# kanster/moped

Hardware: AMD Instinct MI355X
Metric: detections/sec (frames/s) 640x480 ~3k SIFT vs N models (higher is better)
Workload: dtype f32

## Files before the change

moped_amd/csrc/match_screen.hip:

```cpp
#include <type_traits>
#include <hip/hip_fp16.h>

#include <algorithm>
#include <cstdlib>

#include "common.h"
#include "screen.h"

MH_TRACE_TU()

namespace mh {

namespace {

typedef _Float16 half8 __attribute__((ext_vector_type(8)));
typedef float v16f __attribute__((ext_vector_type(16)));
#define MH_AS1 __attribute__((address_space(1)))
#define MH_AS3 __attribute__((address_space(3)))

constexpr int SC_QPAD = 3 * 1024;
constexpr int SC_TILE = 128;
constexpr int SC_TILE_BYTES = SC_TILE * DIM * 2;
constexpr bool SC_SHAPE16_LARGE = true;
constexpr int SC_NW_LARGE = 8;
// ... 141 lines not shown
      const float qq = qnorm[row];
      bad = (!(qq >= 0.f) || qq == __builtin_inff() || !(m < 60000.f)) ? 1 : 0;
      if (qq == -1.f) bad = 2;
      else if (!bad && m == 0.f && qq == 0.f) bad = 3;
    }
    qbad[row] = (uint8_t)bad;
  }
}

constexpr int SC_SLOTS_MAX = 256;
constexpr int SC_SA_SLOTS = 32;
constexpr int SC_SLOT_PITCH = SC_SLOTS_MAX + SC_SA_SLOTS;

#ifdef SC_PROF
__device__ unsigned long long g_sc_prof[8];
__device__ unsigned long long g_sc_trace[2][1024];
static int g_sc_ablate = 0;
#define SC_ABL(bit) ((A.ablate >> (bit)) & 1)
#define SC_EV(e) do { if (tracing && n_ev < 1024) { g_sc_trace[wave >> 2][n_ev++] = ((unsigned long long)(e) << 56) | (__builtin_amdgcn_s_memtime() - t_start); } } while (0)
#else
#define SC_ABL(bit) 0
#define SC_EV(e) do { } while (0)
#endif

struct ScreenArgs {
  const _Float16* qh;
  const _Float16* dbh;
  const float* dneg;
  const float* qnorm;
  const uint8_t* qbad;
  const int32_t* q_count;
  float2* part;
  float* part5;
  const float* tau;
  uint2* recs;
  int32_t* ovf_cnt;
  uint2* ovf;
  int Q, q_pad, ovf_cap, sub_cap;
  int n_sel, tile_first, tile_stride;
  int tiles_base, tiles_rem, n_splits;
  int n_splits_a;
  unsigned pack_keep;
  int skip_first, skip_stride;
  float dmax;
  int ablate;
};
// ... 23 lines not shown
  }
  tau[q] = t;
}

constexpr int SC_TOPK = 4;
constexpr int SC_PART5 = SC_TOPK + 1;
constexpr int SC_SA_SPLITS_MAX = 28;
constexpr int SC_PACK_BITS_MAX = 10;
constexpr float SC_PACK_FLOOR = -1e38f;
constexpr unsigned SC_REC_LAYOUT16 = 0x80000000u;
constexpr unsigned SC_REC_SAMPLE = 0x40000000u;

struct SampleGeom {
  int sa_slots;
  int pack_bits;
  int tile_first, tile_stride, tiles_base, tiles_rem, n_sel;
};

constexpr int HO_PARTS_MAX = 16;
template <int HS>
__global__ __launch_bounds__(64 * HO_PARTS_MAX) void screen_handover_kernel(
    const float* __restrict__ part5, int n_lane_slots, int q_pad, int Q, const int32_t* __restrict__ q_count,
    const float* __restrict__ qnorm, const uint8_t* __restrict__ qbad, float dmax, SampleGeom g, float* __restrict__ tau,
    uint2* __restrict__ recs, unsigned int* __restrict__ inc) {
  MH_TRACE_SCOPE(mh::TK_TAU);
  __shared__ float s_b[HO_PARTS_MAX][64], s_s[HO_PARTS_MAX][64];
  __shared__ int s_cnt[HO_PARTS_MAX][64];
  __shared__ unsigned s_sm[64], s_qm[64];
  const int ql = threadIdx.x, part = threadIdx.y, n_parts = blockDim.y;
  const int q = blockIdx.x * 64 + ql;
  const int Qe = q_count ? min(Q, *q_count) : Q;
  const bool live = q < q_pad && q < Qe && !qbad[q];
  const int ls0 = part * HS;
  float v[HS][SC_PART5];
#pragma unroll
  for (int j = 0; j < HS; ++j)
#pragma unroll
    for (int k = 0; k < SC_PART5; ++k)
      v[j][k] = live && ls0 + j < n_lane_slots ? part5[((size_t)(ls0 + j) * SC_PART5 + k) * q_pad + q] : -__builtin_inff();
  const float qq = live ? qnorm[q] : 0.f;
  if (part == 0) {
    s_sm[ql] = 0u;
    s_qm[ql] = 0u;
  }
  float B = -__builtin_inff(), S = -__builtin_inff();
#pragma unroll
  for (int j = 0; j < HS; ++j) {
// ... 35 lines not shown
#pragma unroll
  for (int j = 0; j < HS; ++j) {
    const int ls = ls0 + j;
    const bool swept = ((sm >> (ls >> 2)) & 1u) && ((qm >> (ls & 3)) & 1u);
    n_j[j] = 0;
    bool run = hand && !swept;
#pragma unroll
    for (int k = 0; k < SC_TOPK; ++k) {
      run = run && v[j][k] > thr;
      n_j[j] += run ? 1 : 0;
    }
    cnt += n_j[j];
  }
  s_cnt[part][ql] = cnt;
  __syncthreads();
  int before = 0, total = 0;
  for (int p = 0; p < n_parts; ++p) {
    const int c = s_cnt[p][ql];
    before += p < part ? c : 0;
    total += c;
  }
  const bool full = total > g.sa_slots;
  if (cnt && !full) {
    uint2* mine = recs + (size_t)q * SC_SLOT_PITCH + SC_SLOTS_MAX + before;
    const unsigned id_mask = (1u << g.pack_bits) - 1u;
    int n = 0;
#pragma unroll
    for (int j = 0; j < HS; ++j) {
      const int split = (ls0 + j) >> 2, quarter = (ls0 + j) & 3;
#pragma unroll
      for (int k = 0; k < SC_TOPK; ++k)
        if (k < n_j[j]) {
          const unsigned id = __float_as_uint(v[j][k]) & id_mask;
          const int sel = split * g.tiles_base + min(split, g.tiles_rem) + (int)(id >> 2);
          const unsigned row0 = (unsigned)((g.tile_first + sel * g.tile_stride) * SC_TILE + (int)(id & 3u) * 32 + 4 * quarter);
          mine[n++] = make_uint2(row0 | SC_REC_LAYOUT16 | SC_REC_SAMPLE, 0xFFu | ((unsigned)screen_record_value(v[j][k], t) << 16));
        }
    }
  }
  if (part == 0 && q < q_pad) {
    if (full) {
      sm = (1u << (n_lane_slots >> 2)) - 1u;
      qm = 0xFu;
    }
    tau[q] = t;
    if (inc) inc[q] = sm ? sm | (qm << 28) : 0u;
  }
}

__device__ __forceinline__ void dma16x4(unsigned voff, const void* b0, const void* b1, const void* b2, const void* b3,
                                        unsigned l0, unsigned l1, unsigned l2, unsigned l3) {
  unsigned keep;
  asm volatile(
      "s_mov_b32 %0, m0\n\t"
      "s_mov_b32 m0, %6\n\ts_nop 0\n\tglobal_load_lds_dwordx4 %1, %2\n\t"
      "s_mov_b32 m0, %7\n\ts_nop 0\n\tglobal_load_lds_dwordx4 %1, %3\n\t"
      "s_mov_b32 m0, %8\n\ts_nop 0\n\tglobal_load_lds_dwordx4 %1, %4\n\t"
      "s_mov_b32 m0, %9\n\ts_nop 0\n\tglobal_load_lds_dwordx4 %1, %5\n\t"
      "s_mov_b32 m0, %0"
      : "=&s"(keep)
      : "v"(voff), "s"(b0), "s"(b1), "s"(b2), "s"(b3), "s"(l0), "s"(l1), "s"(l2), "s"(l3)
      : "memory");
}
__device__ __forceinline__ void dma4(unsigned voff, const void* base, unsigned lds_dst) {
  unsigned keep;
  asm volatile("s_mov_b32 %0, m0\n\ts_mov_b32 m0, %3\n\ts_nop 0\n\tglobal_load_lds_dword %1, %2\n\ts_mov_b32 m0, %0"
               : "=&s"(keep) : "v"(voff), "s"(base), "s"(lds_dst) : "memory");
}
// ... 336 lines not shown
      const int jj = sel_begin - A.skip_first;
      tile_cur = sel_begin + 1 + jj / d;
      gap_cur = d - jj % d;
    }
  }
  auto stage = [&](int tile, int buf) {
    const unsigned char* tb = reinterpret_cast<const unsigned char*>(A.dbh) + (size_t)tile * SC_TILE_BYTES;
    const unsigned l = lds_base + buf * SC_TILE_BYTES + wave * 1024;
    dma16x4(voff, tb, tb + 8192, tb + 16384, tb + 24576, l, l + 8192, l + 16384, l + 24576);
    if (wave < 3)
      dma4(voff_dd, A.dneg + (size_t)tile * SC_DD, lds_base + SC_NBUF * SC_TILE_BYTES + buf * (SC_DD * 4) + wave * 256);
  };
  if (sel_begin < sel_end) stage(tile_cur, 0);
  half8 bq[NQB][2][4];
#pragma unroll
  for (int nb = 0; nb < NQB; ++nb)
#pragma unroll
    for (int tj = 0; tj < 2; ++tj) {
      const _Float16* row = A.qh + (size_t)(q0 + nb * 32 + 16 * tj + l16) * DIM + 8 * quarter;
#pragma unroll
      for (int s = 0; s < 4; ++s) bq[nb][tj][s] = *reinterpret_cast<const half8*>(row + 32 * s);
    }
  float pk[NQB][2][SC_PART5];
  unsigned n_rec[(NQB + 1) / 2] = {};
  float* const tau_lds = reinterpret_cast<float*>(lds + SC_LDS16_TAU) + wave * 128;
#pragma unroll
  for (int nb = 0; nb < NQB; ++nb)
#pragma unroll
    for (int tj = 0; tj < 2; ++tj)
#pragma unroll
      for (int k = 0; k < SC_PART5; ++k) pk[nb][tj][k] = -__builtin_inff();
  if (MODE == 1)
    for (int i = lane; i < QW; i += 64) tau_lds[i] = A.tau[q0 + i];
  __builtin_amdgcn_s_waitcnt(0x0F70);
  __syncthreads();

  uint4* const recbuf = reinterpret_cast<uint4*>(lds + SC_LDS_TILES + wave * (SC_RECBUF16 * SC_REC16_BYTES));
  int n_parked = 0;
  auto record_bits8 = [](const v4f& d0, const v4f& d1, float top, float thr) {
    unsigned bits = 0;
#pragma unroll
    for (int r = 3; r >= 0; --r) bits = __builtin_amdgcn_alignbit(bits, __float_as_uint(thr - d1[r]), 31);
#pragma unroll
    for (int r = 3; r >= 0; --r) bits = __builtin_amdgcn_alignbit(bits, __float_as_uint(thr - d0[r]), 31);
    return (bits & 0xFFu) | ((unsigned)screen_record_value(top, thr) << 16);
  };
  auto emit = [&](const v4f& d0, const v4f& d1, unsigned& nrec_word, int shift, int q, int row0, float top, float thr, int pos) {
    const int nrec = (int)((nrec_word >> shift) & 0xFFu);
    if (nrec < A.sub_cap) {
      const unsigned dst = (unsigned)q * SC_SLOT_PITCH + (4 * split + quarter) * A.sub_cap + nrec;
      nrec_word += 1u << shift;
      if (pos < SC_RECBUF16) {
        uint4* e = recbuf + 3 * pos;
        e[0] = make_uint4(dst, (unsigned)row0, __float_as_uint(thr), __float_as_uint(top));
        e[1] = make_uint4(__float_as_uint(d0[0]), __float_as_uint(d0[1]), __float_as_uint(d0[2]), __float_as_uint(d0[3]));
        e[2] = make_uint4(__float_as_uint(d1[0]), __float_as_uint(d1[1]), __float_as_uint(d1[2]), __float_as_uint(d1[3]));
      } else {
        A.recs[dst] = make_uint2((unsigned)row0 | SC_REC_LAYOUT16, record_bits8(d0, d1, top, thr));
      }
    } else {
      const int opos = atomicAdd(&A.ovf_cnt[q], 1);
      if (opos < A.ovf_cap) A.ovf[(size_t)q * A.ovf_cap + opos] = make_uint2((unsigned)row0 | SC_REC_LAYOUT16, record_bits8(d0, d1, top, thr));
      if (pos < SC_RECBUF16) recbuf[3 * pos] = make_uint4(0xFFFFFFFFu, 0u, 0u, 0u);
    }
  };
  auto emit_block = [&](bool hit0, bool hit1, const v4f (&p)[2][2], int nb, int row0, float m0, float m1, float thr0, float thr1) {
    const unsigned long long h0 = __ballot(hit0), h1 = __ballot(hit1);
    if ((h0 | h1) == 0ull) return;
    if (hit0)
      emit(p[0][0], p[1][0], n_rec[nb >> 1], 16 * (nb & 1), q0 + nb * 32 + l16, row0, m0, thr0,
           n_parked + (int)__builtin_amdgcn_mbcnt_hi((unsigned)(h0 >> 32), __builtin_amdgcn_mbcnt_lo((unsigned)h0, 0u)));
    n_parked += __popcll(h0);
    if (hit1)
      emit(p[0][1], p[1][1], n_rec[nb >> 1], 16 * (nb & 1) + 8, q0 + nb * 32 + 16 + l16, row0, m1, thr1,
           n_parked + (int)__builtin_amdgcn_mbcnt_hi((unsigned)(h1 >> 32), __builtin_amdgcn_mbcnt_lo((unsigned)h1, 0u)));
    n_parked += __popcll(h1);
  };
  auto flush_parked = [&]() {
    __builtin_amdgcn_fence(__ATOMIC_RELEASE, "wavefront");
    __builtin_amdgcn_wave_barrier();
    __builtin_amdgcn_fence(__ATOMIC_ACQUIRE, "wavefront");
    const int n = min(n_parked, SC_RECBUF16);
    for (int j = lane; j < n; j += 64) {
      const uint4 e = recbuf[3 * j];
      if (e.x == 0xFFFFFFFFu) continue;
      const uint4 x0 = recbuf[3 * j + 1], x1 = recbuf[3 * j + 2];
      const v4f d0 = {__uint_as_float(x0.x), __uint_as_float(x0.y), __uint_as_float(x0.z), __uint_as_float(x0.w)};
      const v4f d1 = {__uint_as_float(x1.x), __uint_as_float(x1.y), __uint_as_float(x1.z), __uint_as_float(x1.w)};
      A.recs[e.x] = make_uint2(e.y | SC_REC_LAYOUT16, record_bits8(d0, d1, __uint_as_float(e.w), __uint_as_float(e.z)));
    }
    __builtin_amdgcn_wave_barrier();
    n_parked = 0;
  };

  auto load_rb = [&](const unsigned char* T, int rb, half8 (&a)[2][4]) {
#pragma unroll
    for (int ti = 0; ti < 2; ++ti) {
      const unsigned char* rowp = T + (rb * 32 + 16 * ti + l16) * 256;
#pragma unroll
      for (int s = 0; s < 4; ++s) a[ti][s] = *reinterpret_cast<const half8*>(rowp + (((4 * s + quarter) ^ l16) << 4));
    }
  };
  auto max3 = [](float a, float b, float c) {
    float r;
    asm("v_max3_f32 %0, %1, %2, %3" : "=v"(r) : "v"(a), "v"(b), "v"(c));
    return r;
  };
  auto max8 = [&](const v4f& x, const v4f& y) {
    return max3(max3(max3(x[0], x[1], x[2]), x[3], y[0]), max3(y[1], y[2], y[3]), -__builtin_inff());
  };
  auto max8x2_after_mfma = [](const v4f (&acc)[2][2], float floor, float& m0, float& m1) {
    float t0, t1;
    asm("s_nop 7\n\ts_nop 7\n\t"
// ... 246 lines not shown
  int ovf_cap;
  float dmax;
  const float* tau;
  float spread;
  int32_t* idx1;
  float* d1;
  float* d2;
  unsigned int* stats;
  int32_t zero_idx;
  float zero_d1, zero_d2;
  SampleGeom g;
  const unsigned int* inc;
  unsigned int* inc_count;
  const _Float16* dbh;
  const float* dneg;
};
typedef const __attribute__((address_space(4))) RsArgs* RsArgsPtr;
__device__ __forceinline__ RsArgsPtr rs_args() {
  RsArgsPtr p = (RsArgsPtr)__builtin_amdgcn_kernarg_segment_ptr();
  asm volatile("" : "+s"(p));
  return p;
}

__device__ __forceinline__ void rs_load_slots(const uint2* recs, int n_slots, int sa_slots, int q, int lane, uint2 (&rv)[RS_ITERS]) {
  const uint2* theirs = recs + (size_t)q * SC_SLOT_PITCH;
  const int n_own = n_slots + sa_slots;
#pragma unroll
  for (int it = 0; it < RS_ITERS; ++it) {
    const int j = it * 64 + lane;
    rv[it] = j < n_own ? theirs[j < n_slots ? j : SC_SLOTS_MAX + (j - n_slots)] : make_uint2(0u, 0u);
  }
}
#define RS_CONST(T, p) ((const __attribute__((address_space(4))) T*)(p))
__device__ __forceinline__ RsScalars rs_load_scalars(const uint8_t* qbad, const float* qnorm, const float* tau, const int32_t* ovf_cnt,
                                                     const unsigned int* inc, const float* qn, int q, int lane) {
  RsScalars v;
  v.qv = reinterpret_cast<const float2*>(qn + (size_t)q * DIM)[lane];
  v.n_ovf = RS_CONST(int32_t, ovf_cnt)[q];
  const unsigned w = RS_CONST(unsigned int, inc ? inc : reinterpret_cast<const unsigned int*>(tau))[q];
  v.bad = (RS_CONST(unsigned int, qbad)[q >> 2] >> (8 * (q & 3))) & 0xFFu;
  v.nq = RS_CONST(float, qnorm)[q];
  v.tau_q = RS_CONST(float, tau)[q];
  v.incw = inc ? w : 0u;
  return v;
}

__device__ __forceinline__ void rescore_query(
    int q, int lane, float* q_sw, int* cand_sw, int* samp_sw, int* ncand_sw, int* nsamp_sw, uint2 (&recv)[RS_ITERS], const RsScalars sc, int Qe,
    const float* __restrict__ db, const float* __restrict__ dnorm, int N,
    RowMap rmap, uint2* __restrict__ recs, int n_slots, int32_t* __restrict__ ovf_cnt, uint2* __restrict__ ovf,
    int ovf_cap, float dmax, float spread, int32_t* __restrict__ idx1, float* __restrict__ d1, float* __restrict__ d2,
    unsigned int* __restrict__ stats, int32_t zero_idx, float zero_d1, float zero_d2, SampleGeom g,
    unsigned int* __restrict__ inc_count, const _Float16* __restrict__ dbh, const float* __restrict__ dneg) {
  uint2* mine = recs + (size_t)q * SC_SLOT_PITCH;
  const int n_own = n_slots + g.sa_slots;
  auto slot_at = [&](int j) -> uint2& { return mine[j < n_slots ? j : SC_SLOTS_MAX + (j - n_slots)]; };
  const int bad = sc.bad;
  const float nq = sc.nq;
  const float tau_q = sc.tau_q;
  const int n_ovf = sc.n_ovf;
  const unsigned incw = sc.incw;
  const float2 qv = sc.qv;
  asm volatile("" ::"v"(bad), "v"(nq), "v"(tau_q), "v"(n_ovf), "v"(incw), "v"(qv.x), "v"(qv.y), "s"(Qe));
  if (q >= Qe) {
    if (lane == 0) {
      idx1[q] = -1;
      d1[q] = __builtin_inff();
      d2[q] = __builtin_inff();
    }
    return;
  }
  if (bad == 2) {
    if (lane == 0) {
      idx1[q] = -1;
      d1[q] = __builtin_inff();
      d2[q] = __builtin_inff();
    }
    return;
  }
  if (bad == 3) {
    if (lane == 0) {
      idx1[q] = zero_idx >= 0 ? row_to_global(rmap, zero_idx) : -1;
      d1[q] = zero_d1;
      d2[q] = zero_d2;
      if (stats) stats[3 * q + 2] += 1u;
    }
    return;
  }
  wave_lds_sync();
  if (lane == 0) {
    *ncand_sw = 0;
    *nsamp_sw = 0;
  }
  q_sw[2 * lane] = qv.x;
  q_sw[2 * lane + 1] = qv.y;
  bool brute = n_ovf > ovf_cap || bad == 1;
  int n_cand = 0;
  if (!brute) {
    float l1 = -__builtin_inff(), l2 = -__builtin_inff();
    const float pert = screen_pack_pert(nq, dmax, g.pack_bits);
    auto bounds = [tau_q, spread, N, dmax, pert](uint2 rec, float& lo, float& hi) {
      if (rec.x & SC_REC_SAMPLE) screen_sample_bounds((unsigned short)(rec.y >> 16), tau_q, pert, dmax, lo, hi);
      else screen_record_bounds((unsigned short)(rec.y >> 16), rec.x & 0x3FFFFFFFu, tau_q, spread, N, dmax, lo, hi);
    };
#pragma unroll
    for (int it = 0; it < RS_ITERS; ++it) {
      const int j = it * 64 + lane;
      uint2 rec = recv[it];
      if (j < n_own) {
        if (rec.y) slot_at(j) = make_uint2(0u, 0u);
      } else if (j < n_own + n_ovf) {
        rec = ovf[(size_t)q * ovf_cap + (j - n_own)];
      }
      recv[it] = rec;
      if (rec.y & 0xFFFFu) {
        float lo, hi;
        bounds(rec, lo, hi);
        l2 = fmaxf(l2, fminf(l1, lo));
        l1 = fmaxf(l1, lo);
      }
    }
#pragma unroll
    for (int d = 1; d < 64; d <<= 1) {
      const float o1 = __shfl_xor(l1, d), o2 = __shfl_xor(l2, d);
      l2 = fmaxf(fmaxf(l2, o2), fminf(l1, o1));
      l1 = fmaxf(l1, o1);
    }
    const float keep_from = l2 - screen_margin(nq, dmax);
#pragma unroll
    for (int it = 0; it < RS_ITERS; ++it) {
      const uint2 rec = recv[it];
      unsigned bits = rec.y & 0xFFFFu;
      if (bits) {
        float lo, hi;
        bounds(rec, lo, hi);
        if (hi < keep_from) bits = 0;
      }
      const int hi_stride = (rec.x & 0x80000000u) ? 16 : 8;
      const int row0 = (int)(rec.x & 0x3FFFFFFFu);
      if (bits && (rec.x & SC_REC_SAMPLE)) {
        const int w = atomicAdd(nsamp_sw, 1);
        if (w < SC_SA_SLOTS) samp_sw[w] = row0;
        bits = 0;
      }
      while (bits) {
        const int r = __builtin_ctz(bits);
        bits &= bits - 1;
        const int w = atomicAdd(ncand_sw, 1);
        if (w < RS_MAXC) cand_sw[w] = row0 + (r & 3) + hi_stride * (r >> 2);
      }
    }
    wave_lds_sync();
    const int n_samp = min(*nsamp_sw, SC_SA_SLOTS), n_pad_rows = (N + SC_TILE - 1) / SC_TILE * SC_TILE;
    for (int p = 0; p < n_samp; p += 2) {
      const bool pair = p + 1 < n_samp;
      const int rx = samp_sw[p], ry = samp_sw[pair ? p + 1 : p];
      if (rx + 19 >= n_pad_rows || ry + 19 >= n_pad_rows) continue;
      const v4f w = sample_pair_values(q_sw, dbh, dneg, rx, ry, lane);
      const int grp = lane >> 4;
      if ((lane & 15) == 0 && (grp < 2 || pair)) {
        const int base = (grp < 2 ? rx : ry) + 16 * (grp & 1);
#pragma unroll
        for (int r = 0; r < 4; ++r)
          if (w[r] > tau_q) {
            const int at = atomicAdd(ncand_sw, 1);
            if (at < RS_MAXC) cand_sw[at] = base + r;
          }
      }
    }
    if (n_samp) wave_lds_sync();
    n_cand = *ncand_sw;
    if (n_cand > RS_MAXC) brute = true;
  } else if (n_ovf > ovf_cap) {
    for (int j = lane; j < n_own; j += 64) slot_at(j) = make_uint2(0u, 0u);
  }
  if (n_ovf && lane == 0) ovf_cnt[q] = 0;
  wave_lds_sync();

  Best best = {__builtin_inff(), __builtin_inff(), -1};
  const int n_rows = brute ? N : n_cand;
  if (!brute && n_cand <= 64) {
    const int my_row = lane < n_cand ? cand_sw[lane] : -1;
    const bool my_ok = my_row >= 0 && my_row < N;
    const float my_dn = my_ok ? dnorm[my_row] : 0.f;
    wave_lds_sync();
    float4* stage = reinterpret_cast<float4*>(cand_sw);
    const int n_st = min(n_cand, RS_STAGE);
    const int half = lane >> 5, c = lane & 31;
    float4 v[RS_STAGE / 2];
#pragma unroll
    for (int i = 0; i < RS_STAGE / 2; ++i) {
      const int r = 2 * i + half;
      const int row_r = __shfl(my_row, r);
      v[i] = make_float4(0.f, 0.f, 0.f, 0.f);
      if (r < n_st && row_r >= 0 && row_r < N) v[i] = reinterpret_cast<const float4*>(db + (size_t)row_r * DIM)[c];
    }
// ... 34 lines not shown
          take(best, exact_dist(q_sw, db + (size_t)row * DIM, nq, dnorm[row]), row);
      }
    }
    if (lane == 0 && inc_count) atomicAdd(inc_count, 1u);
  }
#pragma unroll
  for (int d = 1; d < 64; d <<= 1) {
    const float ob1 = __shfl_xor(best.b1, d), ob2 = __shfl_xor(best.b2, d);
    const int oi1 = __shfl_xor(best.i1, d);
    if (oi1 >= 0) merge(best, ob1, ob2, oi1);
  }
  if (lane == 0) {
    idx1[q] = best.i1 >= 0 ? row_to_global(rmap, best.i1) : -1;
    d1[q] = best.b1;
    d2[q] = best.b2;
    if (stats) {
      stats[3 * q] += (unsigned)n_cand;
      stats[3 * q + 1] += brute ? 1u : 0u;
      stats[3 * q + 2] += 1u;
    }
  }
}

template <int WAVES, int PF>
__global__ __launch_bounds__(64 * WAVES) __attribute__((amdgpu_waves_per_eu(WAVES == 12 ? 6 : 8, WAVES == 12 ? 6 : 8))) void rescore_kernel(const RsArgs args) {
  MH_TRACE_SCOPE(mh::TK_PASS_C);
  extern __shared__ __attribute__((aligned(16))) unsigned char rs_lds[];
  const int lane0 = threadIdx.x & 63;
  const int wave0 = __builtin_amdgcn_readfirstlane(threadIdx.x >> 6);
  const int q_first = blockIdx.x * WAVES + wave0, q_stride = (int)gridDim.x * WAVES;
  if (q_first >= args.Q) return;
  const int Qe = args.q_count ? min(args.Q, *RS_CONST(int32_t, args.q_count)) : args.Q;
  uint2 recv_next[RS_ITERS];
  RsScalars sc_next = {};
  if (PF >= 1) rs_load_slots(args.recs, args.n_slots, args.g.sa_slots, q_first, lane0, recv_next);
  if (PF >= 2) sc_next = rs_load_scalars(args.qbad, args.qnorm, args.tau, args.ovf_cnt, args.inc, args.qn, q_first, lane0);
  for (int q = q_first;; q += q_stride) {
    int lane = lane0, wave = wave0;
    asm volatile("" : "+v"(lane), "+s"(wave));
    float* const q_sw = reinterpret_cast<float*>(rs_lds) + wave * DIM;
    int* const cand_sw = reinterpret_cast<int*>(rs_lds + (size_t)WAVES * DIM * 4) + wave * RS_MAXC;
    int* const samp_sw = reinterpret_cast<int*>(rs_lds + (size_t)WAVES * (DIM + RS_MAXC) * 4) + wave * SC_SA_SLOTS;
    int* const ncand_sw = reinterpret_cast<int*>(rs_lds + (size_t)WAVES * (DIM + RS_MAXC + SC_SA_SLOTS) * 4) + wave;
    int* const nsamp_sw = ncand_sw + WAVES;
    const RsArgsPtr A = rs_args();
    const int Q = A->Q;
    if (q >= Q) break;
    uint2 recv[RS_ITERS];
    if (PF >= 1) {
#pragma unroll
      for (int it = 0; it < RS_ITERS; ++it) recv[it] = recv_next[it];
    } else {
      rs_load_slots(A->recs, A->n_slots, A->g.sa_slots, q, lane, recv);
    }
    const RsScalars sc = PF >= 2 ? sc_next : rs_load_scalars(A->qbad, A->qnorm, A->tau, A->ovf_cnt, A->inc, A->qn, q, lane);
    if (PF >= 1 && q + q_stride < Q) {
      rs_load_slots(A->recs, A->n_slots, A->g.sa_slots, q + q_stride, lane, recv_next);
      if (PF >= 2) sc_next = rs_load_scalars(A->qbad, A->qnorm, A->tau, A->ovf_cnt, A->inc, A->qn, q + q_stride, lane);
    }
    RowMap rmap;
    rmap.glo = A->rmap.glo;
    rmap.llo = A->rmap.llo;
    rmap.nb = A->rmap.nb;
    rmap.base = A->rmap.base;
    const SampleGeom g = {A->g.sa_slots, A->g.pack_bits, A->g.tile_first, A->g.tile_stride, A->g.tiles_base, A->g.tiles_rem, A->g.n_sel};
    rescore_query(q, lane, q_sw, cand_sw, samp_sw, ncand_sw, nsamp_sw, recv, sc, Qe, A->db, A->dnorm, A->N, rmap, A->recs,
                  A->n_slots, A->ovf_cnt, A->ovf, A->ovf_cap, A->dmax, A->spread, A->idx1, A->d1, A->d2, A->stats, A->zero_idx,
                  A->zero_d1, A->zero_d2, g, A->inc_count, A->dbh, A->dneg);
  }
}
static_assert(std::is_same<decltype(&rescore_kernel<RS_WAVES, 0>), void (*)(RsArgs)>::value,
              "rs_args() reads RsArgs from offset 0 of the kernel argument segment: it must stay the only parameter");

__global__ __launch_bounds__(64) void screen_values_kernel(const _Float16* __restrict__ qh, const _Float16* __restrict__ dbh,
                                                           const float* __restrict__ dneg, int n_rows, float* __restrict__ out,
                                                           int shape16) {
  const int lane = threadIdx.x, half = lane >> 5, l32 = lane & 31;
  const int q0 = blockIdx.x * 32, r0 = blockIdx.y * 32;
  if (shape16) {
    const int quarter = lane >> 4, l16 = lane & 15;
#pragma unroll
    for (int ti = 0; ti < 2; ++ti)
#pragma unroll
      for (int tj = 0; tj < 2; ++tj) {
        v4f acc;
#pragma unroll
        for (int r = 0; r < 4; ++r) {
          const int row = r0 + 16 * ti + 4 * quarter + r;
          acc[r] = dneg[(size_t)(row >> 7) * SC_DD + (row & 127)];
        }
#pragma unroll
        for (int s = 0; s < 4; ++s) {
          const half8 a = *reinterpret_cast<const half8*>(dbh + (size_t)(r0 + 16 * ti + l16) * DIM + 32 * s + 8 * quarter);
          const half8 b = *reinterpret_cast<const half8*>(qh + (size_t)(q0 + 16 * tj + l16) * DIM + 32 * s + 8 * quarter);
// ... 33 lines not shown
  q_s[2 * lane] = qv.x;
  q_s[2 * lane + 1] = qv.y;
  __syncthreads();
  const v4f w = sample_pair_values(q_s, dbh, dneg, row0[2 * q], row0[2 * q + 1], lane);
  if ((lane & 15) == 0)
#pragma unroll
    for (int r = 0; r < 4; ++r) out[(size_t)q * 16 + 4 * (lane >> 4) + r] = w[r];
}

}

#ifdef SC_PROF
extern "C" int mh_debug_screen_trace(unsigned long long* out ) {
  return hipMemcpyFromSymbol(out, HIP_SYMBOL(g_sc_trace), 2 * 1024 * sizeof(unsigned long long)) == hipSuccess ? 0 : -1;
}
extern "C" int mh_debug_screen_prof(unsigned long long out[8], int reset, int ablate) {
  if (hipMemcpyFromSymbol(out, HIP_SYMBOL(g_sc_prof), 8 * sizeof(unsigned long long)) != hipSuccess) return -1;
  if (reset) {
    unsigned long long z[8] = {};
    if (hipMemcpyToSymbol(HIP_SYMBOL(g_sc_prof), z, sizeof z) != hipSuccess) return -1;
  }
  g_sc_ablate = ablate;
  return 0;
}
#endif

float screen_margin_host(float qq, float dmax) { return screen_margin(qq, dmax); }

size_t screen_db_half_elems(int N) { return ((size_t)N + SC_TILE - 1) / SC_TILE * SC_TILE * DIM; }
size_t screen_dneg_elems(int N) { return ((size_t)N + SC_TILE - 1) / SC_TILE * SC_DD; }

void launch_db_to_half(const float* db, const float* dnorm, int N, _Float16* dbh, float* dneg, unsigned int* stats,
                       hipStream_t s) {
  const size_t n_chunks = screen_db_half_elems(N) / 8;
  if (n_chunks == 0) return;
  const unsigned blocks = (unsigned)std::min<size_t>((n_chunks + 255) / 256, 2048);
  hipLaunchKernelGGL(db_to_half_kernel, dim3(blocks), dim3(256), 0, s, db, dnorm, N, n_chunks, dbh, dneg, stats);
  launch_db_aggregates(dnorm, N, dneg, stats, s);
}

void launch_db_aggregates(const float* dnorm, int N, float* dneg, unsigned int* stats, hipStream_t s) {
  const int n_tiles = (N + SC_TILE - 1) / SC_TILE;
  if (n_tiles == 0) return;
  hipLaunchKernelGGL(db_block_bounds_kernel, dim3((n_tiles * 4 + 255) / 256), dim3(256), 0, s, dnorm, N, n_tiles, dneg, stats);
  hipLaunchKernelGGL(db_zero_query_kernel, dim3(1), dim3(1024), 0, s, dnorm, N, stats);
}
// ... 65 lines not shown
  hipLaunchKernelGGL(screen_tau_kernel, dim3((a.q_pad + 255) / 256), dim3(256), 0, s, a.part, Sa, a.q_pad, a.Q, a.q_count,
                     a.qnorm, a.qbad, a.dmax, const_cast<float*>(a.tau));
  if (ev) hipEventRecord(ev[3], s);
  static const int sb_pin = exp_int("MH_SCREEN_SPLITS_B", 0);
  if (blocks_b <= 0) blocks_b = (long)n_tiles * nqb_e * NW / 8 >= (NQB >= 4 ? 16L : 24L) * 512 ? 512 : 256;
  blocks_b *= 8 / NW;
  const int Sb = sb_pin > 0 ? std::min(std::min(sb_pin, n_tiles), SC_SLOTS_MAX / 2)
                            : splits_for(n_tiles, blocks_b, SC_SLOTS_MAX / 2);
  a.n_sel = n_tiles;
  a.tile_first = 0;
  a.tile_stride = 1;
  a.n_splits = Sb;
  a.tiles_base = n_tiles / Sb;
  a.tiles_rem = n_tiles % Sb;
  a.sub_cap = std::max(1, std::min(48, SC_SLOTS_MAX / (2 * Sb)));
  hipLaunchKernelGGL((screen_kernel<1, NQB, NW>), dim3(nqb * Sb), dim3(SC_THREADS), SC_LDS_BYTES, s, a);
  if (ev) hipEventRecord(ev[4], s);
  *n_slots_out = 2 * Sb * a.sub_cap;
}

struct Plan16 {
  bool onesweep;
  int stride, tile_first, n_sel_a, Sa, pack_bits;
  int n_sel_b, Sb, sub_cap;
};
template <int NQB>
Plan16 plan_passes16(int qe, int n_tiles, int sample, int blocks_a, int blocks_b) {
  constexpr int QB = 32 * NQB * 8;
  const int nqb_e = (qe + QB - 1) / QB;
  auto splits_for = [&](int n_sel, int target, int s_max) {
    int S = std::max(1, target / nqb_e);
    S = std::min(std::min(S, n_sel), s_max);
    if (S >= 8 && (S / 8 * 8) * 33 >= S * 32) S = S / 8 * 8;
    return std::max(S, 1);
  };
  Plan16 p;
  const int every = sample == 8 && n_tiles < 256 ? 4 : sample;
  p.stride = n_tiles >= 4 * every ? every : 1;
  p.n_sel_a = (n_tiles + p.stride - 1) / p.stride;
  p.Sa = splits_for(p.n_sel_a, blocks_a, SC_SA_SPLITS_MAX);
  p.tile_first = std::max(0, std::min(p.stride / 2, n_tiles - 1 - (p.n_sel_a - 1) * p.stride));
  static const int onesweep_on = exp_int("MH_SCREEN_ONESWEEP", 1);
  if (onesweep_on && p.stride > 1)
    while (4 * ((p.n_sel_a + p.Sa - 1) / p.Sa) > (1 << SC_PACK_BITS_MAX) && p.Sa < SC_SA_SPLITS_MAX) ++p.Sa;
  const int blocks_slot = 4 * ((p.n_sel_a + p.Sa - 1) / p.Sa);
  int bits = 2;
  while ((1 << bits) < blocks_slot) ++bits;
  p.onesweep = onesweep_on && p.stride > 1 && bits <= SC_PACK_BITS_MAX;
  p.pack_bits = p.onesweep ? bits : 0;
  constexpr int SB16_MAX = SC_SLOTS_MAX / 12;
  static_assert(SC_SLOTS_MAX / 4 < 256, "a sub-list's record count must fit the byte screen16_kernel keeps it in");
  p.n_sel_b = p.onesweep ? n_tiles - p.n_sel_a : n_tiles;
  p.Sb = 1;
  if (blocks_b > 0) {
    p.Sb = std::min(splits_for(p.n_sel_b, blocks_b, SC_SLOTS_MAX / 4), SB16_MAX);
  } else {
    double best = 1e30;
    for (int c = 1; c <= std::min(SB16_MAX, std::max(1, p.n_sel_b / 8)); ++c) {
      const double cost = (double)((nqb_e * c + 255) / 256) * (double)((p.n_sel_b + c - 1) / c);
      if (cost <= best) {
        best = cost;
        p.Sb = c;
      }
    }
  }
  const int slots_target = n_tiles >= 2048 ? SC_SLOTS_MAX : (n_tiles >= 512 ? 160 : 96);
  p.sub_cap = std::max(1, std::min(std::max(3, (slots_target + 4 * p.Sb - 1) / (4 * p.Sb)), SC_SLOTS_MAX / (4 * p.Sb)));
  return p;
}

template <int NQB>
void launch_passes16(ScreenArgs a, int Q, int qe, int n_tiles, int sample, int blocks_a, int blocks_b, int* n_slots_out,
                     SampleGeom* geom_out, unsigned int* inc, hipEvent_t* ev, hipStream_t s) {
  constexpr int QB = 32 * NQB * 8;
  static DynLds attr0, attr1;
  attr0.ensure(screen16_kernel<0, NQB>, SC_LDS16_BYTES);
  attr1.ensure(screen16_kernel<1, NQB>, SC_LDS16_BYTES);
  const int nqb = (Q + QB - 1) / QB;
  const Plan16 p = plan_passes16<NQB>(qe, n_tiles, sample, blocks_a, blocks_b);
  a.n_sel = p.n_sel_a;
  a.tile_first = p.tile_first;
  a.tile_stride = p.stride;
  a.n_splits = p.Sa;
  a.tiles_base = p.n_sel_a / p.Sa;
  a.tiles_rem = p.n_sel_a % p.Sa;
  a.n_splits_a = p.Sa;
  a.pack_keep = ~((1u << p.pack_bits) - 1u);
  a.skip_first = a.skip_stride = 0;
  hipLaunchKernelGGL((screen16_kernel<0, NQB>), dim3(nqb * p.Sa), dim3(512), SC_LDS16_BYTES, s, a);
  if (ev) hipEventRecord(ev[2], s);
  SampleGeom g = {p.onesweep ? SC_SA_SLOTS : 0, p.pack_bits, a.tile_first, a.tile_stride, a.tiles_base, a.tiles_rem, a.n_sel};
  static_assert(SC_SA_SPLITS_MAX <= 2 * HO_PARTS_MAX, "a thread of screen_handover_kernel holds at most 8 lane slots");
  if (p.Sa <= HO_PARTS_MAX)
    hipLaunchKernelGGL(screen_handover_kernel<4>, dim3((a.q_pad + 63) / 64), dim3(64, p.Sa), 0, s, (const float*)a.part5, 4 * p.Sa,
                       a.q_pad, a.Q, a.q_count, a.qnorm, a.qbad, a.dmax, g, const_cast<float*>(a.tau), a.recs, inc);
  else
    hipLaunchKernelGGL(screen_handover_kernel<8>, dim3((a.q_pad + 63) / 64), dim3(64, (p.Sa + 1) / 2), 0, s, (const float*)a.part5,
                       4 * p.Sa, a.q_pad, a.Q, a.q_count, a.qnorm, a.qbad, a.dmax, g, const_cast<float*>(a.tau), a.recs, inc);
#ifdef MH_EXPERIMENTS
  if (exp_int("MH_SCREEN_NO_HITS", 0)) hipMemsetAsync(const_cast<float*>(a.tau), 0x7f, (size_t)a.q_pad * sizeof(float), s);
#endif
  if (ev) hipEventRecord(ev[3], s);
  a.n_sel = p.n_sel_b;
  a.tile_first = 0;
  a.tile_stride = 1;
  a.skip_first = p.onesweep ? p.tile_first : 0;
  a.skip_stride = p.onesweep ? p.stride : 0;
  a.n_splits = p.Sb;
  a.tiles_base = p.n_sel_b / p.Sb;
  a.tiles_rem = p.n_sel_b % p.Sb;
  a.sub_cap = p.sub_cap;
  hipLaunchKernelGGL((screen16_kernel<1, NQB>), dim3(nqb * p.Sb), dim3(512), SC_LDS16_BYTES, s, a);
  if (ev) hipEventRecord(ev[4], s);
  *n_slots_out = 4 * p.Sb * a.sub_cap;
  *geom_out = g;
}

template <int WAVES, int PF>
void launch_pass_c(int grid, hipStream_t s, const RsArgs& args) {
  static DynLds attr;
  attr.ensure(rescore_kernel<WAVES, PF>, rs_lds_bytes(WAVES));
  hipLaunchKernelGGL((rescore_kernel<WAVES, PF>), dim3(grid), dim3(64 * WAVES), rs_lds_bytes(WAVES), s, args);
}

struct ShapeChoice {
  int nqb_sel;
  bool passes16;
};
ShapeChoice choose_shape(int qe, int n_tiles) {
  static const int nqb_pin = exp_int("MH_SCREEN_NQB", 0);
  int nqb_sel = qe > 640 ? 2 : 1;
  if (qe >= 2048 && (long)n_tiles * ((qe + 1023) / 1024) >= 16L * 256) nqb_sel = 4;
  if (nqb_pin >= 1 && nqb_pin <= 4) nqb_sel = nqb_pin;
  static const int shape_pin = exp_int("MH_SCREEN_SHAPE", 0);
  const bool shape16 = shape_pin == 2 || (shape_pin == 0 && SC_SHAPE16_LARGE);
  const bool p16 = shape16 && ((nqb_sel == 4 && (shape_pin == 2 || (qe + 1023) / 1024 >= 12)) || (nqb_sel == 2 && shape_pin == 2));
  return {nqb_sel, p16};
}

int screen_sample_every() {
  static const int sample = std::max(1, exp_int("MH_SCREEN_SAMPLE", 8));
  return sample;
}

}
// ... 67 lines not shown
  else if (nqb_sel == 4 && nw_sel == 4) launch_passes<4, 4>(a, Q, qe, n_tiles, sample, blocks_a, blocks_b, &n_slots, sb.ev, sbig, 256);
  else if (nqb_sel == 4) launch_passes<4, 8>(a, Q, qe, n_tiles, sample, blocks_a, blocks_b, &n_slots, sb.ev, sbig, 256);
  else if (nqb_sel == 3) launch_passes<3, 8>(a, Q, qe, n_tiles, sample, blocks_a, blocks_b, &n_slots, sb.ev, sbig, 256);
  else if (nqb_sel == 2 && nw_sel == 4) launch_passes<2, 4>(a, Q, qe, n_tiles, sample, blocks_a, blocks_b, &n_slots, sb.ev, sbig, 256);
  else if (nqb_sel == 2) launch_passes<2, 8>(a, Q, qe, n_tiles, sample, blocks_a, blocks_b, &n_slots, sb.ev, sbig, 256);
  else launch_passes<1, 8>(a, Q, qe, n_tiles, sample, blocks_a, blocks_b, &n_slots, sb.ev, sbig, 256);
  if (sbig != s) {
    hipEventRecord(sb.ev_out, sbig);
    hipStreamWaitEvent(s, sb.ev_out, 0);
  }
  RsArgs ca;
  ca.qn = qn; ca.qnorm = qnorm; ca.qbad = sb.qbad; ca.Q = Q; ca.q_count = q_count; ca.db = db; ca.dnorm = dnorm; ca.N = N;
  ca.rmap = rmap; ca.recs = sb.recs; ca.n_slots = n_slots; ca.ovf_cnt = sb.ovf_cnt; ca.ovf = sb.ovf; ca.ovf_cap = sb.ovf_cap;
  ca.dmax = sdb.dmax; ca.tau = sb.tau; ca.spread = sdb.spread; ca.idx1 = idx1; ca.d1 = d1; ca.d2 = d2; ca.stats = sb.stats;
  ca.zero_idx = sdb.zero_idx; ca.zero_d1 = sdb.zero_d1; ca.zero_d2 = sdb.zero_d2; ca.g = geom;
  ca.inc = geom.sa_slots > 0 ? sb.inc : nullptr; ca.inc_count = sb.inc ? sb.inc + sb.q_pad : nullptr; ca.dbh = sdb.dbh; ca.dneg = sdb.dneg;
#ifdef MH_EXPERIMENTS
  static const int pc_waves = exp_int("MH_PASSC_WAVES", RS_WAVES), pc_k = exp_int("MH_PASSC_K", RS_FAT_K);
  static const int pc_pf = exp_int("MH_PASSC_PREFETCH", 0), pc_all = exp_int("MH_PASSC_FAT_ALL", 0);
  const int n_cus = sb.n_cus > 0 ? sb.n_cus : 256;
  const int fat_waves = pc_waves == 12 ? 12 : RS_WAVES_FAT;
  if (pc_waves != RS_WAVES && (pc_all || Q > RS_FAT_K * n_cus * RS_WAVES_FAT)) {
    const int cover = (Q + fat_waves - 1) / fat_waves, grid = pc_k > 0 ? std::min(cover, pc_k * n_cus) : cover;
    if (fat_waves == 12 && pc_pf == 0) launch_pass_c<12, 0>(grid, s, ca);
    else if (fat_waves == 12 && pc_pf == 1) launch_pass_c<12, 1>(grid, s, ca);
    else if (fat_waves == 12) launch_pass_c<12, 2>(grid, s, ca);
    else if (pc_pf == 0) launch_pass_c<RS_WAVES_FAT, 0>(grid, s, ca);
    else if (pc_pf == 1) launch_pass_c<RS_WAVES_FAT, 1>(grid, s, ca);
    else launch_pass_c<RS_WAVES_FAT, 2>(grid, s, ca);
  } else
#endif
  launch_pass_c<RS_WAVES, 0>((Q + RS_WAVES - 1) / RS_WAVES, s, ca);
  if (sb.ev) hipEventRecord(sb.ev[5], s);
}

}
```

Before: 16640.

## Replace fixed per-split record sub-lists with atomic-counted compact per-query lists

The 16-row screen pass no longer writes hit records into fixed per-split sub-slots tracked by packed byte counters. Each hit is instead appended to a contiguous per-query list through an atomic counter, which the handover kernel seeds with its sample records. The rescore kernel gets a COMPACT variant that reads only the counted records, usually one 64-wide load, instead of scanning every sub-slot plus an overflow region. This trades per-record global atomics in the flush for fewer slot loads and zeroing in pass C. It also drops the sub_cap sizing logic.

```diff
diff --git a/moped_amd/csrc/match_screen.hip b/moped_amd/csrc/match_screen.hip
--- a/moped_amd/csrc/match_screen.hip
+++ b/moped_amd/csrc/match_screen.hip
@@ -187,6 +187,9 @@
 #define SC_ABL(bit) 0
 #define SC_EV(e) do { } while (0)
 #endif
+#ifdef MH_EXPERIMENTS
+__device__ unsigned long long g_sc_direct_appends;
+#endif
 
 struct ScreenArgs {
   const _Float16* qh;
@@ -256,7 +259,7 @@
 __global__ __launch_bounds__(64 * HO_PARTS_MAX) void screen_handover_kernel(
     const float* __restrict__ part5, int n_lane_slots, int q_pad, int Q, const int32_t* __restrict__ q_count,
     const float* __restrict__ qnorm, const uint8_t* __restrict__ qbad, float dmax, SampleGeom g, float* __restrict__ tau,
-    uint2* __restrict__ recs, unsigned int* __restrict__ inc) {
+    uint2* __restrict__ recs, int32_t* __restrict__ rec_cnt, unsigned int* __restrict__ inc) {
   MH_TRACE_SCOPE(mh::TK_TAU);
   __shared__ float s_b[HO_PARTS_MAX][64], s_s[HO_PARTS_MAX][64];
   __shared__ int s_cnt[HO_PARTS_MAX][64];
@@ -338,7 +341,7 @@
   }
   const bool full = total > g.sa_slots;
   if (cnt && !full) {
-    uint2* mine = recs + (size_t)q * SC_SLOT_PITCH + SC_SLOTS_MAX + before;
+    uint2* mine = recs + (size_t)q * SC_SLOT_PITCH + before;
     const unsigned id_mask = (1u << g.pack_bits) - 1u;
     int n = 0;
 #pragma unroll
@@ -360,6 +363,7 @@
       qm = 0xFu;
     }
     tau[q] = t;
+    rec_cnt[q] = full ? 0 : total;
     if (inc) inc[q] = sm ? sm | (qm << 28) : 0u;
   }
 }
@@ -742,7 +746,6 @@
       for (int s = 0; s < 4; ++s) bq[nb][tj][s] = *reinterpret_cast<const half8*>(row + 32 * s);
     }
   float pk[NQB][2][SC_PART5];
-  unsigned n_rec[(NQB + 1) / 2] = {};
   float* const tau_lds = reinterpret_cast<float*>(lds + SC_LDS16_TAU) + wave * 128;
 #pragma unroll
   for (int nb = 0; nb < NQB; ++nb)
@@ -765,34 +768,34 @@
     for (int r = 3; r >= 0; --r) bits = __builtin_amdgcn_alignbit(bits, __float_as_uint(thr - d0[r]), 31);
     return (bits & 0xFFu) | ((unsigned)screen_record_value(top, thr) << 16);
   };
-  auto emit = [&](const v4f& d0, const v4f& d1, unsigned& nrec_word, int shift, int q, int row0, float top, float thr, int pos) {
-    const int nrec = (int)((nrec_word >> shift) & 0xFFu);
-    if (nrec < A.sub_cap) {
-      const unsigned dst = (unsigned)q * SC_SLOT_PITCH + (4 * split + quarter) * A.sub_cap + nrec;
-      nrec_word += 1u << shift;
-      if (pos < SC_RECBUF16) {
-        uint4* e = recbuf + 3 * pos;
-        e[0] = make_uint4(dst, (unsigned)row0, __float_as_uint(thr), __float_as_uint(top));
-        e[1] = make_uint4(__float_as_uint(d0[0]), __float_as_uint(d0[1]), __float_as_uint(d0[2]), __float_as_uint(d0[3]));
-        e[2] = make_uint4(__float_as_uint(d1[0]), __float_as_uint(d1[1]), __float_as_uint(d1[2]), __float_as_uint(d1[3]));
-      } else {
-        A.recs[dst] = make_uint2((unsigned)row0 | SC_REC_LAYOUT16, record_bits8(d0, d1, top, thr));
-      }
+  auto append = [&](int q, int at, unsigned row0, unsigned bits) {
+    if (at < SC_SLOT_PITCH) A.recs[(size_t)q * SC_SLOT_PITCH + at] = make_uint2(row0 | SC_REC_LAYOUT16, bits);
+  };
+  auto emit = [&](const v4f& d0, const v4f& d1, int q, int row0, float top, float thr, int pos) {
+    if (pos < SC_RECBUF16) {
+      uint4* e = recbuf + 3 * pos;
+      e[0] = make_uint4((unsigned)q, (unsigned)row0, __float_as_uint(thr), __float_as_uint(top));
+      e[1] = make_uint4(__float_as_uint(d0[0]), __float_as_uint(d0[1]), __float_as_uint(d0[2]), __float_as_uint(d0[3]));
+      e[2] = make_uint4(__float_as_uint(d1[0]), __float_as_uint(d1[1]), __float_as_uint(d1[2]), __float_as_uint(d1[3]));
     } else {
-      const int opos = atomicAdd(&A.ovf_cnt[q], 1);
-      if (opos < A.ovf_cap) A.ovf[(size_t)q * A.ovf_cap + opos] = make_uint2((unsigned)row0 | SC_REC_LAYOUT16, record_bits8(d0, d1, top, thr));
-      if (pos < SC_RECBUF16) recbuf[3 * pos] = make_uint4(0xFFFFFFFFu, 0u, 0u, 0u);
+#ifdef MH_EXPERIMENTS
+      atomicAdd(&g_sc_direct_appends, 1ull);
+#endif
+      const int at = atomicAdd(&A.ovf_cnt[q], 1);
+      int qa = q;
+      asm volatile("" : "+v"(qa));
+      append(qa, at, (unsigned)row0, record_bits8(d0, d1, top, thr));
     }
   };
   auto emit_block = [&](bool hit0, bool hit1, const v4f (&p)[2][2], int nb, int row0, float m0, float m1, float thr0, float thr1) {
     const unsigned long long h0 = __ballot(hit0), h1 = __ballot(hit1);
     if ((h0 | h1) == 0ull) return;
     if (hit0)
-      emit(p[0][0], p[1][0], n_rec[nb >> 1], 16 * (nb & 1), q0 + nb * 32 + l16, row0, m0, thr0,
+      emit(p[0][0], p[1][0], q0 + nb * 32 + l16, row0, m0, thr0,
            n_parked + (int)__builtin_amdgcn_mbcnt_hi((unsigned)(h0 >> 32), __builtin_amdgcn_mbcnt_lo((unsigned)h0, 0u)));
     n_parked += __popcll(h0);
     if (hit1)
-      emit(p[0][1], p[1][1], n_rec[nb >> 1], 16 * (nb & 1) + 8, q0 + nb * 32 + 16 + l16, row0, m1, thr1,
+      emit(p[0][1], p[1][1], q0 + nb * 32 + 16 + l16, row0, m1, thr1,
            n_parked + (int)__builtin_amdgcn_mbcnt_hi((unsigned)(h1 >> 32), __builtin_amdgcn_mbcnt_lo((unsigned)h1, 0u)));
     n_parked += __popcll(h1);
   };
@@ -800,15 +803,29 @@
     __builtin_amdgcn_fence(__ATOMIC_RELEASE, "wavefront");
     __builtin_amdgcn_wave_barrier();
     __builtin_amdgcn_fence(__ATOMIC_ACQUIRE, "wavefront");
+    constexpr int TRIPS = (SC_RECBUF16 + 63) / 64;
     const int n = min(n_parked, SC_RECBUF16);
-    for (int j = lane; j < n; j += 64) {
-      const uint4 e = recbuf[3 * j];
-      if (e.x == 0xFFFFFFFFu) continue;
-      const uint4 x0 = recbuf[3 * j + 1], x1 = recbuf[3 * j + 2];
-      const v4f d0 = {__uint_as_float(x0.x), __uint_as_float(x0.y), __uint_as_float(x0.z), __uint_as_float(x0.w)};
-      const v4f d1 = {__uint_as_float(x1.x), __uint_as_float(x1.y), __uint_as_float(x1.z), __uint_as_float(x1.w)};
-      A.recs[e.x] = make_uint2(e.y | SC_REC_LAYOUT16, record_bits8(d0, d1, __uint_as_float(e.w), __uint_as_float(e.z)));
-    }
+    uint4 e[TRIPS];
+    int at[TRIPS];
+#pragma unroll
+    for (int i = 0; i < TRIPS; ++i) {
+      e[i] = make_uint4(0u, 0u, 0u, 0u);
+      if (lane + 64 * i < n) e[i] = recbuf[3 * (lane + 64 * i)];
+    }
+#pragma unroll
+    for (int i = 0; i < TRIPS; ++i) {
+      at[i] = SC_SLOT_PITCH;
+      if (lane + 64 * i < n) at[i] = atomicAdd(&A.ovf_cnt[e[i].x], 1);
+    }
+#pragma unroll
+    for (int i = 0; i < TRIPS; ++i)
+      if (at[i] < SC_SLOT_PITCH) {
+        const int j = lane + 64 * i;
+        const uint4 x0 = recbuf[3 * j + 1], x1 = recbuf[3 * j + 2];
+        const v4f d0 = {__uint_as_float(x0.x), __uint_as_float(x0.y), __uint_as_float(x0.z), __uint_as_float(x0.w)};
+        const v4f d1 = {__uint_as_float(x1.x), __uint_as_float(x1.y), __uint_as_float(x1.z), __uint_as_float(x1.w)};
+        append((int)e[i].x, at[i], e[i].y, record_bits8(d0, d1, __uint_as_float(e[i].w), __uint_as_float(e[i].z)));
+      }
     __builtin_amdgcn_wave_barrier();
     n_parked = 0;
   };
@@ -1101,8 +1118,16 @@
   return p;
 }
 
+constexpr int RS_ITERS_C = (SC_SLOT_PITCH + 63) / 64;
+template <int COMPACT>
 __device__ __forceinline__ void rs_load_slots(const uint2* recs, int n_slots, int sa_slots, int q, int lane, uint2 (&rv)[RS_ITERS]) {
   const uint2* theirs = recs + (size_t)q * SC_SLOT_PITCH;
+  if (COMPACT) {
+    rv[0] = theirs[lane];
+#pragma unroll
+    for (int it = 1; it < RS_ITERS; ++it) rv[it] = make_uint2(0u, 0u);
+    return;
+  }
   const int n_own = n_slots + sa_slots;
 #pragma unroll
   for (int it = 0; it < RS_ITERS; ++it) {
@@ -1124,6 +1149,8 @@
   return v;
 }
 
+static_assert(RS_ITERS_C <= RS_ITERS, "a counted list's slots fit the registers the scan has");
+template <int COMPACT>
 __device__ __forceinline__ void rescore_query(
     int q, int lane, float* q_sw, int* cand_sw, int* samp_sw, int* ncand_sw, int* nsamp_sw, uint2 (&recv)[RS_ITERS], const RsScalars sc, int Qe,
     const float* __restrict__ db, const float* __restrict__ dnorm, int N,
@@ -1132,8 +1159,8 @@
     unsigned int* __restrict__ stats, int32_t zero_idx, float zero_d1, float zero_d2, SampleGeom g,
     unsigned int* __restrict__ inc_count, const _Float16* __restrict__ dbh, const float* __restrict__ dneg) {
   uint2* mine = recs + (size_t)q * SC_SLOT_PITCH;
-  const int n_own = n_slots + g.sa_slots;
-  auto slot_at = [&](int j) -> uint2& { return mine[j < n_slots ? j : SC_SLOTS_MAX + (j - n_slots)]; };
+  const int n_own = COMPACT ? min(sc.n_ovf, SC_SLOT_PITCH) : n_slots + g.sa_slots;
+  auto slot_at = [&](int j) -> uint2& { return mine[COMPACT || j < n_slots ? j : SC_SLOTS_MAX + (j - n_slots)]; };
   const int bad = sc.bad;
   const float nq = sc.nq;
   const float tau_q = sc.tau_q;
@@ -1173,7 +1200,7 @@
   }
   q_sw[2 * lane] = qv.x;
   q_sw[2 * lane + 1] = qv.y;
-  bool brute = n_ovf > ovf_cap || bad == 1;
+  bool brute = n_ovf > (COMPACT ? SC_SLOT_PITCH : ovf_cap) || bad == 1;
   int n_cand = 0;
   if (!brute) {
     float l1 = -__builtin_inff(), l2 = -__builtin_inff();
@@ -1182,11 +1209,21 @@
       if (rec.x & SC_REC_SAMPLE) screen_sample_bounds((unsigned short)(rec.y >> 16), tau_q, pert, dmax, lo, hi);
       else screen_record_bounds((unsigned short)(rec.y >> 16), rec.x & 0x3FFFFFFFu, tau_q, spread, N, dmax, lo, hi);
     };
-#pragma unroll
-    for (int it = 0; it < RS_ITERS; ++it) {
+    const bool more = COMPACT && n_own > 64;
+    if (more) {
+#pragma unroll
+      for (int it = 1; it < RS_ITERS_C; ++it) {
+        const int j = it * 64 + lane;
+        recv[it] = j < n_own ? mine[j] : make_uint2(0u, 0u);
+      }
+    }
+    auto scan = [&](int it) {
       const int j = it * 64 + lane;
       uint2 rec = recv[it];
-      if (j < n_own) {
+      if (COMPACT) {
+        if (j < n_own) mine[j] = make_uint2(0u, 0u);
+        else rec = make_uint2(0u, 0u);
+      } else if (j < n_own) {
         if (rec.y) slot_at(j) = make_uint2(0u, 0u);
       } else if (j < n_own + n_ovf) {
         rec = ovf[(size_t)q * ovf_cap + (j - n_own)];
@@ -1198,6 +1235,16 @@
         l2 = fmaxf(l2, fminf(l1, lo));
         l1 = fmaxf(l1, lo);
       }
+    };
+    if (COMPACT) {
+      scan(0);
+      if (more) {
+#pragma unroll
+        for (int it = 1; it < RS_ITERS_C; ++it) scan(it);
+      }
+    } else {
+#pragma unroll
+      for (int it = 0; it < RS_ITERS; ++it) scan(it);
     }
 #pragma unroll
     for (int d = 1; d < 64; d <<= 1) {
@@ -1206,8 +1253,7 @@
       l1 = fmaxf(l1, o1);
     }
     const float keep_from = l2 - screen_margin(nq, dmax);
-#pragma unroll
-    for (int it = 0; it < RS_ITERS; ++it) {
+    auto keep = [&](int it) {
       const uint2 rec = recv[it];
       unsigned bits = rec.y & 0xFFFFu;
       if (bits) {
@@ -1228,6 +1274,16 @@
         const int w = atomicAdd(ncand_sw, 1);
         if (w < RS_MAXC) cand_sw[w] = row0 + (r & 3) + hi_stride * (r >> 2);
       }
+    };
+    if (COMPACT) {
+      keep(0);
+      if (more) {
+#pragma unroll
+        for (int it = 1; it < RS_ITERS_C; ++it) keep(it);
+      }
+    } else {
+#pragma unroll
+      for (int it = 0; it < RS_ITERS; ++it) keep(it);
     }
     wave_lds_sync();
     const int n_samp = min(*nsamp_sw, SC_SA_SLOTS), n_pad_rows = (N + SC_TILE - 1) / SC_TILE * SC_TILE;
@@ -1250,7 +1306,7 @@
     if (n_samp) wave_lds_sync();
     n_cand = *ncand_sw;
     if (n_cand > RS_MAXC) brute = true;
-  } else if (n_ovf > ovf_cap) {
+  } else if (COMPACT ? n_ovf > 0 : n_ovf > ovf_cap) {
     for (int j = lane; j < n_own; j += 64) slot_at(j) = make_uint2(0u, 0u);
   }
   if (n_ovf && lane == 0) ovf_cnt[q] = 0;
@@ -1331,7 +1387,7 @@
   }
 }
 
-template <int WAVES, int PF>
+template <int WAVES, int PF, int COMPACT>
 __global__ __launch_bounds__(64 * WAVES) __attribute__((amdgpu_waves_per_eu(WAVES == 12 ? 6 : 8, WAVES == 12 ? 6 : 8))) void rescore_kernel(const RsArgs args) {
   MH_TRACE_SCOPE(mh::TK_PASS_C);
   extern __shared__ __attribute__((aligned(16))) unsigned char rs_lds[];
@@ -1342,7 +1398,7 @@
   const int Qe = args.q_count ? min(args.Q, *RS_CONST(int32_t, args.q_count)) : args.Q;
   uint2 recv_next[RS_ITERS];
   RsScalars sc_next = {};
-  if (PF >= 1) rs_load_slots(args.recs, args.n_slots, args.g.sa_slots, q_first, lane0, recv_next);
+  if (PF >= 1) rs_load_slots<COMPACT>(args.recs, args.n_slots, args.g.sa_slots, q_first, lane0, recv_next);
   if (PF >= 2) sc_next = rs_load_scalars(args.qbad, args.qnorm, args.tau, args.ovf_cnt, args.inc, args.qn, q_first, lane0);
   for (int q = q_first;; q += q_stride) {
     int lane = lane0, wave = wave0;
@@ -1360,11 +1416,11 @@
 #pragma unroll
       for (int it = 0; it < RS_ITERS; ++it) recv[it] = recv_next[it];
     } else {
-      rs_load_slots(A->recs, A->n_slots, A->g.sa_slots, q, lane, recv);
+      rs_load_slots<COMPACT>(A->recs, A->n_slots, A->g.sa_slots, q, lane, recv);
     }
     const RsScalars sc = PF >= 2 ? sc_next : rs_load_scalars(A->qbad, A->qnorm, A->tau, A->ovf_cnt, A->inc, A->qn, q, lane);
     if (PF >= 1 && q + q_stride < Q) {
-      rs_load_slots(A->recs, A->n_slots, A->g.sa_slots, q + q_stride, lane, recv_next);
+      rs_load_slots<COMPACT>(A->recs, A->n_slots, A->g.sa_slots, q + q_stride, lane, recv_next);
       if (PF >= 2) sc_next = rs_load_scalars(A->qbad, A->qnorm, A->tau, A->ovf_cnt, A->inc, A->qn, q + q_stride, lane);
     }
     RowMap rmap;
@@ -1373,12 +1429,12 @@
     rmap.nb = A->rmap.nb;
     rmap.base = A->rmap.base;
     const SampleGeom g = {A->g.sa_slots, A->g.pack_bits, A->g.tile_first, A->g.tile_stride, A->g.tiles_base, A->g.tiles_rem, A->g.n_sel};
-    rescore_query(q, lane, q_sw, cand_sw, samp_sw, ncand_sw, nsamp_sw, recv, sc, Qe, A->db, A->dnorm, A->N, rmap, A->recs,
+    rescore_query<COMPACT>(q, lane, q_sw, cand_sw, samp_sw, ncand_sw, nsamp_sw, recv, sc, Qe, A->db, A->dnorm, A->N, rmap, A->recs,
                   A->n_slots, A->ovf_cnt, A->ovf, A->ovf_cap, A->dmax, A->spread, A->idx1, A->d1, A->d2, A->stats, A->zero_idx,
                   A->zero_d1, A->zero_d2, g, A->inc_count, A->dbh, A->dneg);
   }
 }
-static_assert(std::is_same<decltype(&rescore_kernel<RS_WAVES, 0>), void (*)(RsArgs)>::value,
+static_assert(std::is_same<decltype(&rescore_kernel<RS_WAVES, 0, 0>), void (*)(RsArgs)>::value,
               "rs_args() reads RsArgs from offset 0 of the kernel argument segment: it must stay the only parameter");
 
 __global__ __launch_bounds__(64) void screen_values_kernel(const _Float16* __restrict__ qh, const _Float16* __restrict__ dbh,
@@ -1458,6 +1514,14 @@
   }
   g_sc_ablate = ablate;
   return 0;
+}
+#endif
+#ifdef MH_EXPERIMENTS
+extern "C" long long mh_debug_screen_direct_appends(int reset) {
+  unsigned long long v = 0, z = 0;
+  if (hipMemcpyFromSymbol(&v, HIP_SYMBOL(g_sc_direct_appends), sizeof v) != hipSuccess) return -1;
+  if (reset && hipMemcpyToSymbol(HIP_SYMBOL(g_sc_direct_appends), &z, sizeof z) != hipSuccess) return -1;
+  return (long long)v;
 }
 #endif
 
@@ -1569,7 +1633,7 @@
 struct Plan16 {
   bool onesweep;
   int stride, tile_first, n_sel_a, Sa, pack_bits;
-  int n_sel_b, Sb, sub_cap;
+  int n_sel_b, Sb;
 };
 template <int NQB>
 Plan16 plan_passes16(int qe, int n_tiles, int sample, int blocks_a, int blocks_b) {
@@ -1596,7 +1660,6 @@
   p.onesweep = onesweep_on && p.stride > 1 && bits <= SC_PACK_BITS_MAX;
   p.pack_bits = p.onesweep ? bits : 0;
   constexpr int SB16_MAX = SC_SLOTS_MAX / 12;
-  static_assert(SC_SLOTS_MAX / 4 < 256, "a sub-list's record count must fit the byte screen16_kernel keeps it in");
   p.n_sel_b = p.onesweep ? n_tiles - p.n_sel_a : n_tiles;
   p.Sb = 1;
   if (blocks_b > 0) {
@@ -1611,8 +1674,6 @@
       }
     }
   }
-  const int slots_target = n_tiles >= 2048 ? SC_SLOTS_MAX : (n_tiles >= 512 ? 160 : 96);
-  p.sub_cap = std::max(1, std::min(std::max(3, (slots_target + 4 * p.Sb - 1) / (4 * p.Sb)), SC_SLOTS_MAX / (4 * p.Sb)));
   return p;
 }
 
@@ -1640,10 +1701,10 @@
   static_assert(SC_SA_SPLITS_MAX <= 2 * HO_PARTS_MAX, "a thread of screen_handover_kernel holds at most 8 lane slots");
   if (p.Sa <= HO_PARTS_MAX)
     hipLaunchKernelGGL(screen_handover_kernel<4>, dim3((a.q_pad + 63) / 64), dim3(64, p.Sa), 0, s, (const float*)a.part5, 4 * p.Sa,
-                       a.q_pad, a.Q, a.q_count, a.qnorm, a.qbad, a.dmax, g, const_cast<float*>(a.tau), a.recs, inc);
+                       a.q_pad, a.Q, a.q_count, a.qnorm, a.qbad, a.dmax, g, const_cast<float*>(a.tau), a.recs, a.ovf_cnt, inc);
   else
     hipLaunchKernelGGL(screen_handover_kernel<8>, dim3((a.q_pad + 63) / 64), dim3(64, (p.Sa + 1) / 2), 0, s, (const float*)a.part5,
-                       4 * p.Sa, a.q_pad, a.Q, a.q_count, a.qnorm, a.qbad, a.dmax, g, const_cast<float*>(a.tau), a.recs, inc);
+                       4 * p.Sa, a.q_pad, a.Q, a.q_count, a.qnorm, a.qbad, a.dmax, g, const_cast<float*>(a.tau), a.recs, a.ovf_cnt, inc);
 #ifdef MH_EXPERIMENTS
   if (exp_int("MH_SCREEN_NO_HITS", 0)) hipMemsetAsync(const_cast<float*>(a.tau), 0x7f, (size_t)a.q_pad * sizeof(float), s);
 #endif
@@ -1656,18 +1717,22 @@
   a.n_splits = p.Sb;
   a.tiles_base = p.n_sel_b / p.Sb;
   a.tiles_rem = p.n_sel_b % p.Sb;
-  a.sub_cap = p.sub_cap;
   hipLaunchKernelGGL((screen16_kernel<1, NQB>), dim3(nqb * p.Sb), dim3(512), SC_LDS16_BYTES, s, a);
   if (ev) hipEventRecord(ev[4], s);
-  *n_slots_out = 4 * p.Sb * a.sub_cap;
+  *n_slots_out = 0;
   *geom_out = g;
 }
 
+template <int WAVES, int PF, int COMPACT>
+void launch_pass_c_layout(int grid, hipStream_t s, const RsArgs& args) {
+  static DynLds attr;
+  attr.ensure(rescore_kernel<WAVES, PF, COMPACT>, rs_lds_bytes(WAVES));
+  hipLaunchKernelGGL((rescore_kernel<WAVES, PF, COMPACT>), dim3(grid), dim3(64 * WAVES), rs_lds_bytes(WAVES), s, args);
+}
 template <int WAVES, int PF>
-void launch_pass_c(int grid, hipStream_t s, const RsArgs& args) {
-  static DynLds attr;
-  attr.ensure(rescore_kernel<WAVES, PF>, rs_lds_bytes(WAVES));
-  hipLaunchKernelGGL((rescore_kernel<WAVES, PF>), dim3(grid), dim3(64 * WAVES), rs_lds_bytes(WAVES), s, args);
+void launch_pass_c(int grid, hipStream_t s, const RsArgs& args, bool compact) {
+  if (compact) launch_pass_c_layout<WAVES, PF, 1>(grid, s, args);
+  else launch_pass_c_layout<WAVES, PF, 0>(grid, s, args);
 }
 
 struct ShapeChoice {
@@ -1781,15 +1846,15 @@
   const int fat_waves = pc_waves == 12 ? 12 : RS_WAVES_FAT;
   if (pc_waves != RS_WAVES && (pc_all || Q > RS_FAT_K * n_cus * RS_WAVES_FAT)) {
     const int cover = (Q + fat_waves - 1) / fat_waves, grid = pc_k > 0 ? std::min(cover, pc_k * n_cus) : cover;
-    if (fat_waves == 12 && pc_pf == 0) launch_pass_c<12, 0>(grid, s, ca);
-    else if (fat_waves == 12 && pc_pf == 1) launch_pass_c<12, 1>(grid, s, ca);
-    else if (fat_waves == 12) launch_pass_c<12, 2>(grid, s, ca);
-    else if (pc_pf == 0) launch_pass_c<RS_WAVES_FAT, 0>(grid, s, ca);
-    else if (pc_pf == 1) launch_pass_c<RS_WAVES_FAT, 1>(grid, s, ca);
-    else launch_pass_c<RS_WAVES_FAT, 2>(grid, s, ca);
+    if (fat_waves == 12 && pc_pf == 0) launch_pass_c<12, 0>(grid, s, ca, shape.passes16);
+    else if (fat_waves == 12 && pc_pf == 1) launch_pass_c<12, 1>(grid, s, ca, shape.passes16);
+    else if (fat_waves == 12) launch_pass_c<12, 2>(grid, s, ca, shape.passes16);
+    else if (pc_pf == 0) launch_pass_c<RS_WAVES_FAT, 0>(grid, s, ca, shape.passes16);
+    else if (pc_pf == 1) launch_pass_c<RS_WAVES_FAT, 1>(grid, s, ca, shape.passes16);
+    else launch_pass_c<RS_WAVES_FAT, 2>(grid, s, ca, shape.passes16);
   } else
 #endif
-  launch_pass_c<RS_WAVES, 0>((Q + RS_WAVES - 1) / RS_WAVES, s, ca);
+  launch_pass_c<RS_WAVES, 0>((Q + RS_WAVES - 1) / RS_WAVES, s, ca, shape.passes16);
   if (sb.ev) hipEventRecord(sb.ev[5], s);
 }
 
```

New measurement: 16890, median of 6. 1.01x the previous value.
